# verdurin/pbdagcon

Hardware: AMD Instinct MI355X
Metric: consensus bases/sec (whole node) (higher is better)
Workload: dtype u8

## Files before the change

pbdagcon_amd/csrc/k_build.hip.h:

```cpp
#pragma once
#include <hip/hip_runtime.h>
#include "dagcon_dev.h"
#include "k_norm_run.hip.h"
#include "k_norm_fin.hip.h"

#define DG_WAVE 64
#ifndef DG_LPW
#define DG_LPW 8u
#endif

__device__ __forceinline__ bool dg_failed(const DgParams &p) {
    return __hip_atomic_load(&p.st->err_flags, __ATOMIC_RELAXED, __HIP_MEMORY_SCOPE_AGENT) != 0;
}
__device__ __forceinline__ void dg_fail(const DgParams &p, uint32_t bit) {
    atomicOr(&p.st->err_flags, bit);
}
__device__ __forceinline__ void dg_fail_target(const DgParams &p, uint32_t t, uint32_t bit) {
    atomicOr(&p.tfail[t], bit);
}
__device__ __forceinline__ bool dg_tskip(const DgParams &p, uint32_t t) {
    return !p.tactive[t] || __hip_atomic_load(&p.tfail[t], __ATOMIC_RELAXED, __HIP_MEMORY_SCOPE_AGENT) != 0;
}
__device__ __forceinline__ bool dg_askip(const DgParams &p, uint32_t a) {
    return !(p.flags & DG_F_A1_ONLY) && __hip_atomic_load(&p.tfail[p.aln_tgt[a]], __ATOMIC_RELAXED, __HIP_MEMORY_SCOPE_AGENT) != 0;
// ... 697 lines not shown
    if (p.emit_scan) {
        for (unsigned long long m = __ballot(pfx_entry); m; m = __ballot(pfx_entry)) {
            const uint32_t pp = (uint32_t)__builtin_amdgcn_readlane((int)prev_pos, __ffsll((long long)m) - 1);
            const uint32_t x = rvalid ? Cm[pp] : 0u;
            const uint32_t e = dg_wave_excl(x, lane);
            if (pfx_entry && prev_pos == pp) { prev = gbase[pp] + e + x - 1u; pfx_entry = false; }
        }
    }
    uint32_t c_base = 0x80000000u;
#define DG_STAGE(I)                                                                         \
    do {                                                                                    \
        c_base = (I) & ~7u;                                                                 \
        const uint4 *src_ = reinterpret_cast<const uint4 *>(buf + c_base);                  \
        uint4 v_[DG_ECOLS / 8];                                                             \
        _Pragma("unroll") for (int k_ = 0; k_ < (int)(DG_ECOLS / 8); k_++)                  \
            v_[k_] = (c_base + 8u * k_ < hi) ? src_[k_] : make_uint4(0, 0, 0, 0);           \
        _Pragma("unroll") for (int k_ = 0; k_ < (int)(DG_ECOLS / 8); k_++) {                \
            uint32_t *dst_ = reinterpret_cast<uint32_t *>(colw) + 4 * k_;                   \
            dst_[0] = v_[k_].x; dst_[1] = v_[k_].y; dst_[2] = v_[k_].z; dst_[3] = v_[k_].w; \
        }                                                                                   \
    } while (0)
#define DG_COLUMN(I, OUT)                                                                   \
    do {                                                                                    \
        if ((I) - c_base >= DG_ECOLS) DG_STAGE(I);                                          \
        OUT = colw[(I) - c_base];                                                           \
    } while (0)
#define DG_DEPART(NXT)                                                       \
    do {                                                                     \
        if (!(fl & DG_EF_OWN)) break;                                        \
        if (fl & DG_EF_BB) {                                                 \
            if (prev_pos >= pos0) s_D[(prev_pos - pos0) * 64 + lane] = (NXT) + 1u;   \
            else DG_ECELL(Dm, prev_pos) = (NXT) + 1u;                \
        } else {                                                             \
            const uint32_t _rk = prev - prev_pos;                            \
            DG_EPW(3u * _rk) = (NXT);                                        \
            DG_EPW(3u * _rk + 1u) = 1u;                                      \
        }                                                                    \
    } while (0)

    uint32_t pos0 = P0;
    while (pos0 < P1 && (pos0 <= blen || (!__all(bbpos == DG_EDONE) && pos0 <= blen + 2u * DG_EB))) {
        uint32_t bidv[DG_EB];
        {
            const uint4 *bp = reinterpret_cast<const uint4 *>(bid + pos0);
#pragma unroll
            for (int k = 0; k < DG_EB / 4; k++) {
                const uint4 v = bp[k];
                bidv[4 * k] = v.x; bidv[4 * k + 1] = v.y; bidv[4 * k + 2] = v.z; bidv[4 * k + 3] = v.w;
            }
        }
        uint32_t gbv[DG_EB], cmv[DG_EB];
        {
            const uint4 *gp = reinterpret_cast<const uint4 *>(gbase + pos0);
#pragma unroll
            for (int k = 0; k < DG_EB / 4; k++) {
                const uint4 v = gp[k];
                gbv[4 * k] = v.x; gbv[4 * k + 1] = v.y; gbv[4 * k + 2] = v.z; gbv[4 * k + 3] = v.w;
            }
            if constexpr (sizeof(CT) == 1) {
                const uint2 v = *reinterpret_cast<const uint2 *>(Cm + pos0);
#pragma unroll
                for (int k = 0; k < 8; k++) cmv[k] = ((k < 4 ? v.x : v.y) >> (8 * (k & 3))) & 0xFFu;
            } else {
                const uint4 *cp = reinterpret_cast<const uint4 *>(Cm + pos0);
#pragma unroll
                for (int k = 0; k < DG_EB / 4; k++) {
                    const uint4 v = cp[k];
                    cmv[4 * k] = v.x; cmv[4 * k + 1] = v.y; cmv[4 * k + 2] = v.z; cmv[4 * k + 3] = v.w;
                }
            }
        }
        if (p.emit_scan) {
#pragma unroll
            for (int j = 0; j < DG_EB; j++) {
                const uint32_t x = rvalid ? cmv[j] : 0u;
                cmv[j] = __ballot(x != 0u) ? dg_wave_excl(x, lane) : 0u;
            }
        }
        if (bbpos != DG_EDONE && i < hi && (i - c_base) + DG_ENEED > DG_ECOLS) DG_STAGE(i);
        uint32_t acell[DG_EB];
#pragma unroll
        for (int j = 0; j < DG_EB; j++) { acell[j] = 0; s_D[j * 64 + lane] = 0; }
        uint32_t exit_val = 0;
#pragma unroll
        for (int j = 0; j < DG_EB; j++) {
            const uint32_t pos = pos0 + j;
            uint32_t f_apos = 0, f_key = 0, f_first = 0;
            asm volatile("" : "+v"(fl));
            if (bbpos == pos && pos < P1) {
                uint32_t ins_id = 0;
                uint32_t kacc = 0;
                uint16_t c = 0;
                f_apos = prev_pos;
                const bool f_anc_ok = fl == (DG_EF_BB | DG_EF_OWN) && pos - prev_pos < 16u;
                for (;;) {
                    if (i < hi) DG_COLUMN(i, c);
                    const uint8_t qb = DG_Q(c), tb = DG_T(c);
                    if (i >= hi || qb == tb || qb == DG_GAP) break;
                    if (tb == DG_GAP) {
                        if (!ins_id) { ins_id = gbv[j] + cmv[j]; f_first = ins_id; }
                        kacc = (kacc << 8) | qb;
                        const uint32_t id = ins_id++;
                        const uint32_t rk = id - bbpos;
                        DgNode nd;
                        nd.out_len = 1; nd.in_len = 1; nd.base = qb; nd.flags = 0; nd.pad = 0;
                        nd.weight = 1; nd.pending = 1;
                        nd.out_off = 3u * rk; nd.in_off = 3u * rk + 2u; nd.out_cap = 1; nd.in_cap = 1;
                        nd.bbpos = (int32_t)bbpos;
                        *reinterpret_cast<DgNode *>(reinterpret_cast<char *>(ndt) + (id << 5)) = nd;
                        DG_EPW(3u * rk + 2u) = prev;
                        DG_DEPART(id);
                        prev = id; prev_pos = bbpos; fl = DG_EF_OWN;
                    }
                    i++;
                }
                if (i >= hi) {
                    exit_val = (fl & DG_EF_OWN) ? prev + 1u : 0u;
                    const uint32_t ex = bid[exitpos];
                    DG_DEPART(ex);
                    bbpos = DG_EDONE;
                } else {
                    const uint8_t qb = DG_Q(c), tb = DG_T(c);
                    if (qb == tb) {
                        const uint32_t cur = bidv[j];
                        acell[j] = ((uint32_t)tb << 25) | (prev + 1u);
                        if (f_anc_ok && kacc != 0u && kacc < (1u << 24)) f_key = kacc | ((pos - f_apos) << 24);
                        DG_DEPART(cur);
                        prev = cur; prev_pos = bbpos; fl = DG_EF_BB | DG_EF_OWN;
                    } else {
                        acell[j] = ((uint32_t)tb << 25) | DG_CELL_DEL;
                    }
                    bbpos++;
                    i++;
                }
            }
            if (p.fold) {
                const unsigned long long em = __ballot(f_key != 0u);
                if (em & (em - 1ull)) {
                    uint32_t fn;
                    const uint32_t vic = dg_emit_fold(em, f_key, f_first, pos, ndt, pool, &fn, lane);
                    if (vic | fn) {
                        const uint32_t dv = vic ? 0u : (f_first + 1u) | ((fn - 1u) << 25);
                        if (f_apos >= pos0) s_D[(f_apos - pos0) * 64 + lane] = dv;
                        if (f_apos < pos0 || f_apos == 0u) DG_ECELL(Dm, f_apos) = dv;
                        if (vic) acell[j] = (acell[j] & 0xFE000000u) | DG_CELL_DUP;
                    }
                }
            }
        }
        if (r < K && lane < DG_ERPW) {
#pragma unroll
            for (int j = 0; j < DG_EB; j++) {
                const uint32_t pos = pos0 + j;
                if (pos <= blen && pos >= P0 && pos < P1) {
                    DG_ECELL(Am, pos) = acell[j];
                    const uint32_t dv = s_D[j * 64 + lane];
                    if (pos > 0 || dv) DG_ECELL(Dm, pos) = dv;
                }
            }
            if (exit_val) DG_ECELL(Am, exitpos) = exit_val;
        }
        pos0 += DG_EB;
    }
    {
        const bool ahead = bbpos != DG_EDONE && (fl & DG_EF_OWN);
        uint32_t q = bbpos, nxt = 0;
        bool found = false, pfx_next = false;
        if (ahead) {
            while (i < hi) {
                const uint16_t c = buf[i];
                const uint8_t qb = DG_Q(c), tb = DG_T(c);
                if (qb == tb) { nxt = bid[q]; found = true; break; }
                if (qb == DG_GAP) { q++; i++; continue; }
                if (tb == DG_GAP) {
                    if (p.emit_scan) pfx_next = true; else nxt = gbase[q] + Cm[q];
                    found = true; break;
                }
                i++;
            }
        }
        if (p.emit_scan) {
            for (unsigned long long m = __ballot(pfx_next); m; m = __ballot(pfx_next)) {
                const uint32_t pp = (uint32_t)__builtin_amdgcn_readlane((int)q, __ffsll((long long)m) - 1);
                const uint32_t x = rvalid ? Cm[pp] : 0u;
                const uint32_t e = dg_wave_excl(x, lane);
                if (pfx_next && q == pp) { nxt = gbase[pp] + e; pfx_next = false; }
            }
        }
        if (ahead) {
            if (!found) {
                nxt = bid[exitpos];
                Am[(uint64_t)exitpos * K + r] = prev + 1u;
            }
            const uint32_t pos0 = 0xFFFFFFFFu;
            DG_DEPART(nxt);
        }
    }
#undef DG_EPW
#undef DG_ECELL
#undef DG_DEPART
#undef DG_COLUMN
#undef DG_STAGE
}

#include "k_lists_row.hip.h"
__device__ __forceinline__ int dg_lds_find(volatile int32_t *vals, int n, int x, int lane) {
    for (int b = 0; b < n; b += DG_WAVE) {
        int i = b + lane;
        bool hit = (i < n) && (vals[i] == x);
        unsigned long long m = __ballot(hit);
        if (m) return b + (__ffsll((long long)m) - 1);
    }
    return -1;
}

__device__ __forceinline__ uint32_t dg_pool_alloc(const DgParams &p, uint32_t t, uint32_t words, int lane) {
    uint32_t off = 0;
    if (lane == 0) {
        t = (uint32_t)__builtin_amdgcn_readfirstlane((int)t);
        off = atomicAdd(&p.pool_top[t], words);
        if ((uint64_t)off + words > p.pool_size[t]) { dg_fail(p, DG_E_POOL_TGT); p.st->bad_target = t; off = 0xFFFFFFFFu; }
    }
    return (uint32_t)__builtin_amdgcn_readlane((int)off, 0);
}

__device__ __forceinline__ unsigned long long dg_list_row(int32_t val, int32_t extra, int32_t chain, int32_t ulo, int32_t uhi,
                                                          int lane, int32_t &cnt, unsigned long long &cm) {
    cm = __ballot(val == chain);
    const bool uniq = val >= ulo && val < uhi;
    unsigned long long firsts = __ballot(uniq);
    cnt = 1 + extra;
    unsigned long long rem = __ballot(val != 0 && !uniq) & ~cm;
    while (rem) {
        const int first = __ffsll((long long)rem) - 1;
        const int32_t x = __builtin_amdgcn_readlane(val, first);
        const unsigned long long same = __ballot(val == x);
        rem &= ~same;
        if (lane == first) cnt = __popcll(same) + extra;
        firsts |= 1ull << first;
    }
    return firsts;
}

struct DgPosLists { uint32_t o_len, o_off, o_cap, i_len, i_off, i_cap, cov; };

__device__ __forceinline__ bool dg_lists_pos(const DgParams &p, uint32_t t, uint32_t *pool, uint32_t pos, uint32_t blen,
                                             uint32_t capb, uint32_t fixed0, int lane, bool do_out, bool do_in,
                                             uint32_t dep, uint32_t arr, int32_t v1, int32_t chain_o, int32_t ulo_o,
                                             int32_t chain_i, int32_t ulo_i, DgPosLists &r) {
#define DG_LPOOL(OFF) (*reinterpret_cast<uint32_t *>(reinterpret_cast<char *>(pool) + (((uint32_t)(OFF)) << 2)))
    if (do_out) {
        const int32_t val = (int32_t)DG_CELL_ID(dep), extra = (int32_t)(dep >> 25);
        int32_t cnt;
        unsigned long long cm;
        const unsigned long long firsts = dg_list_row(val, extra, chain_o, ulo_o, chain_o, lane, cnt, cm);
        const uint32_t n = 1u + (uint32_t)__popcll(firsts);
        uint32_t off = fixed0 + pos * 3u * capb, cap = capb;
        if (n > capb) {
            cap = n + 2u;
            off = dg_pool_alloc(p, t, 2u * cap, lane);
            if (off == 0xFFFFFFFFu) return false;
        }
        const uint32_t idx = 1u + (uint32_t)__popcll(firsts & ((1ull << lane) - 1ull));
        if (lane == 0) { DG_LPOOL(off) = (uint32_t)(chain_o - 1); DG_LPOOL(off + 1) = (uint32_t)__popcll(cm); }
        if ((firsts >> lane) & 1ull) { DG_LPOOL(off + 2 * idx) = (uint32_t)(val - 1); DG_LPOOL(off + 2 * idx + 1) = (uint32_t)cnt; }
        r.o_len = n; r.o_off = off; r.o_cap = cap;
    }
    if (do_in) {
        const uint32_t idf = DG_CELL_ID(arr);
        r.cov = 0;
        if (pos <= blen) {
            const unsigned long long covered = __ballot(arr != 0u);
            const uint32_t n_cov = (uint32_t)__popcll(covered);
            const uint32_t n_match = (uint32_t)__popcll(__ballot(arr != 0u && idf != DG_CELL_DEL));
            const uint32_t last_base = covered ? DG_CELL_BASE((uint32_t)__builtin_amdgcn_readlane((int)arr, 63 - __clzll((long long)covered))) : 0u;
            r.cov = n_cov | n_match << 8 | last_base << 16;
        }
        const int32_t val = (arr != 0u && idf != DG_CELL_DEL && idf != DG_CELL_DUP) ? (int32_t)idf : 0;
        int32_t cnt;
        unsigned long long cm;
        const unsigned long long firsts = dg_list_row(val, 0, chain_i, ulo_i, v1, lane, cnt, cm);
        const uint32_t n = 1u + (uint32_t)__popcll(firsts);
        uint32_t off = fixed0 + pos * 3u * capb + 2u * capb, cap = capb;
        if (n > capb) {
            cap = n + 2u;
            off = dg_pool_alloc(p, t, cap, lane);
            if (off == 0xFFFFFFFFu) return false;
        }
        const uint32_t idx = 1u + (uint32_t)__popcll(firsts & ((1ull << lane) - 1ull));
        if (lane == 0) DG_LPOOL(off) = (uint32_t)(chain_i - 1);
        if ((firsts >> lane) & 1ull) DG_LPOOL(off + idx) = (uint32_t)(val - 1);
        r.i_len = n; r.i_off = off; r.i_cap = cap;
    }
#undef DG_LPOOL
    return true;
}

__device__ __forceinline__ uint32_t dg_pool_alloc_lane(const DgParams &p, uint32_t t, uint32_t words) {
    const uint32_t off = atomicAdd(&p.pool_top[t], words);
    if ((uint64_t)off + words > p.pool_size[t]) { dg_fail(p, DG_E_POOL_TGT); p.st->bad_target = t; return 0xFFFFFFFFu; }
    return off;
}

__device__ __forceinline__ void dg_stage_rows(uint32_t *rows, const uint32_t *blk, uint32_t nrows, uint32_t K, uint32_t S,
                                              int lane) {
    if (K == 0) return;
    const uint32_t total = nrows * K, q = DG_WAVE / K, rm = DG_WAVE % K;
    uint32_t row = (uint32_t)lane / K, col = (uint32_t)lane % K;
#pragma unroll 4
    for (uint32_t i = (uint32_t)lane; i < total; i += DG_WAVE) {
        rows[row * S + col] = blk[i];
        row += q; col += rm;
        if (col >= K) { col -= K; row++; }
    }
}

#define DG_LL_WAVES 2u

__global__ __launch_bounds__(64 * DG_LL_WAVES) void k_lists_lanes(DgParams p) {
    extern __shared__ uint32_t s_rows[];
    const uint32_t t = blockIdx.x;
    if (dg_failed(p) || dg_tskip(p, t)) return;
    const uint32_t K = (uint32_t)(p.aln_begin[t + 1] - p.aln_begin[t]);
    if (K > DG_WAVE) return;
    const uint32_t blen = p.tlen[t];
    const int lane = threadIdx.x & 63;
    const uint32_t wave = (uint32_t)__builtin_amdgcn_readfirstlane((int)(threadIdx.x >> 6));
    const uint32_t pos0 = (blockIdx.y * DG_LL_WAVES + wave) * DG_WAVE;
    if (pos0 >= blen + 2) return;
    const uint32_t nrows = min((uint32_t)DG_WAVE, blen + 2 - pos0);
    const uint32_t S = K | 1u;
    uint32_t *rows = s_rows + wave * DG_WAVE * (min(p.max_k, (uint32_t)DG_WAVE) | 1u);
    uint32_t *row = rows + (uint32_t)lane * S;
    const uint64_t nb = p.node_base[t];
    const uint64_t bv = p.bbv_base[t];
    const uint32_t capb = dg_capb(K);
    const uint32_t fixed0 = 3u * p.t_nins[t];
    uint32_t *pool = p.pool + p.pool_base[t];
    const uint32_t *Db = p.matD + p.mat_base[t] + (uint64_t)pos0 * K, *Ab = p.matA + p.mat_base[t] + (uint64_t)pos0 * K;

    const uint32_t pos = pos0 + (uint32_t)lane;
    const bool act = (uint32_t)lane < nrows;
    const bool do_out = act && pos <= blen, do_in = act && pos >= 1;
    const uint32_t b0 = act ? p.bid[bv + pos] : 0u;
    const uint32_t bm = do_in ? p.bid[bv + pos - 1] : 0u;
    const uint32_t bp = do_out ? p.bid[bv + pos + 1] : 0u;
    const uint32_t g0 = act ? p.gbase[bv + pos] : 0u;
    const uint32_t g1 = do_out ? p.gbase[bv + pos + 1] : 0u;
    uint32_t out_len = 0, in_len = 0, r_cov = 0;
    uint32_t r_out = fixed0 + pos * 3u * capb, r_in = r_out + 2u * capb;
    uint32_t out_cap = capb, in_cap = capb;
    bool dead = false;

    dg_stage_rows(rows, Db, nrows, K, S, lane);
    __builtin_amdgcn_fence(__ATOMIC_SEQ_CST, "workgroup");
    DgLaneRow so = {};
    if (do_out) {
        so = dg_lane_row<false>(row, K, bp + 1u, g1 + 1u, bp + 1u);
        if (!so.overflow) {
            if (so.n > capb) {
                const uint32_t off = dg_pool_alloc_lane(p, t, 2u * (so.n + 2u));
                if (off == 0xFFFFFFFFu) dead = true;
                else { r_out = off; out_cap = so.n + 2u; }
            }
            if (!dead) { pool[r_out] = bp; pool[r_out + 1u] = so.c0; out_len = so.n; }
        }
    }
    for (uint32_t j = 1; __ballot(j < out_len) != 0ull; j++)
        if (j < out_len) {
            const uint32_t e = row[j - 1u];
            pool[r_out + 2u * j] = DG_CELL_ID(e) - 1u;
            pool[r_out + 2u * j + 1u] = dg_lane_count(so, e);
        }
    __builtin_amdgcn_fence(__ATOMIC_SEQ_CST, "workgroup");

    dg_stage_rows(rows, Ab, nrows, K, S, lane);
    __builtin_amdgcn_fence(__ATOMIC_SEQ_CST, "workgroup");
    DgLaneRow si = {};
    if (do_in) {
        si = dg_lane_row<true>(row, K, bm + 1u, g0 + 1u, b0 + 1u);
        if (pos <= blen) r_cov = si.n_cov | si.n_match << 8 | si.last_base << 16;
        if (!si.overflow && !dead) {
            if (si.n > capb) {
                const uint32_t off = dg_pool_alloc_lane(p, t, si.n + 2u);
                if (off == 0xFFFFFFFFu) dead = true;
                else { r_in = off; in_cap = si.n + 2u; }
            }
            if (!dead) { pool[r_in] = bm; in_len = si.n; }
        }
    }
    for (uint32_t j = 1; __ballot(j < in_len) != 0ull; j++)
        if (j < in_len) pool[r_in + j] = DG_CELL_ID(row[j - 1u]) - 1u;

    const unsigned long long redo_o = __ballot(do_out && so.overflow != 0u), redo_i = __ballot(do_in && si.overflow != 0u);
    for (unsigned long long rem = redo_o | redo_i; rem; rem &= rem - 1ull) {
        const int pi = __ffsll((long long)rem) - 1;
        const bool ro = (redo_o >> pi) & 1ull, ri = (redo_i >> pi) & 1ull;
        const bool rl = (uint32_t)lane < K;
        const uint32_t dep = rl && ro ? Db[(uint32_t)pi * K + (uint32_t)lane] : 0u;
        const uint32_t arr = rl && ri ? Ab[(uint32_t)pi * K + (uint32_t)lane] : 0u;
        DgPosLists r;
        const bool ok = dg_lists_pos(p, t, pool, pos0 + (uint32_t)pi, blen, capb, fixed0, lane, ro, ri, dep, arr,
                                     __builtin_amdgcn_readlane((int)b0, pi) + 1,
                                     __builtin_amdgcn_readlane((int)bp, pi) + 1, __builtin_amdgcn_readlane((int)g1, pi) + 1,
                                     __builtin_amdgcn_readlane((int)bm, pi) + 1, __builtin_amdgcn_readlane((int)g0, pi) + 1, r);
        if (lane == pi) {
            if (!ok) dead = true;
            else {
                if (ro) { out_len = r.o_len; r_out = r.o_off; out_cap = r.o_cap; }
                if (ri) { in_len = r.i_len; r_in = r.i_off; in_cap = r.i_cap; r_cov = r.cov; }
            }
        }
        if (!ok) break;
    }

    if (act && !dead) {
        const bool inner = pos >= 1 && pos <= blen;
        const uint32_t n_cov = r_cov & 0xFFu, n_match = (r_cov >> 8) & 0xFFu;
        uint32_t base;
        if (pos == 0) base = '^';
        else if (pos == blen + 1) base = '$';
        else if (n_cov) base = r_cov >> 16;
        else base = p.bb ? p.bb[p.bb_off[t] + (pos - 1)] : (uint8_t)'N';
        uint4 *rec = reinterpret_cast<uint4 *>(p.nodes + nb + b0);
        rec[0] = make_uint4(out_len | in_len << 16, base | DG_NF_BACKBONE << 8,
                            inner ? 1u + n_match : 0u,
                            in_len);
        rec[1] = make_uint4(r_out, r_in, out_cap | in_cap << 16, inner ? pos : 0u);
        p.cov[bv + pos] = inner ? (int32_t)n_cov : 0;
    }
}

__global__ __launch_bounds__(256) void k_lists(DgParams p) {
    extern __shared__ int32_t s_tmp[];
    const uint32_t t = blockIdx.x;
    if (dg_failed(p) || dg_tskip(p, t)) return;
    const int lane = threadIdx.x & 63, wave = threadIdx.x >> 6;
    const uint32_t blen = p.tlen[t];
    const uint32_t K = (uint32_t)(p.aln_begin[t + 1] - p.aln_begin[t]);
    if (K <= DG_WAVE) return;
    const uint32_t stride = p.max_k + 2;
    volatile int32_t *vals = s_tmp + (size_t)wave * 2 * stride;
    volatile int32_t *cnts = vals + stride;
    const uint64_t nb = p.node_base[t];
    const uint64_t bv = p.bbv_base[t];
    uint32_t *pool = p.pool + p.pool_base[t];
    const uint32_t *Am0 = p.matA + p.mat_base[t], *Dm0 = p.matD + p.mat_base[t];
    const uint32_t capb = dg_capb(K);
    const uint32_t fixed0 = 3u * p.t_nins[t];
    for (uint32_t pi = 0; pi < DG_LPW; pi++) {
    const uint32_t pos = (blockIdx.y * 4 + wave) * DG_LPW + pi;
    if (pos >= blen + 2) return;
    const uint32_t v = p.bid[bv + pos];
    const uint32_t *Am = Am0 + (uint64_t)pos * K;
    const uint32_t *Dm = Dm0 + (uint64_t)pos * K;
    const uint32_t fixed = fixed0 + pos * 3u * capb;
    uint32_t out_off = fixed, in_off = fixed + 2u * capb;
    uint32_t out_cap = capb, in_cap = capb;
    uint32_t out_len = 0, in_len = 0;
    uint32_t n_match = 0, n_cov = 0, last_base = 0;

    for (int dir = 0; dir < 2; dir++) {
        if (dir == 0 && pos == blen + 1) continue;
        if (dir == 1 && pos == 0) continue;
        const uint32_t *row = dir == 0 ? Dm : Am;
        int n = 1;
        int32_t lv = dir == 0 ? (int32_t)p.bid[bv + pos + 1] : (int32_t)p.bid[bv + pos - 1];
        int32_t lc = 0;
        bool in_lds = false;
        for (uint32_t r0 = 0; r0 < K; r0 += DG_WAVE) {
            const uint32_t r = r0 + lane;
            const uint32_t cell = r < K ? row[r] : 0u;
            int32_t val = (int32_t)DG_CELL_ID(cell);
            const int32_t extra = dir == 0 ? (int32_t)(cell >> 25) : 0;
            if (dir == 1) {
                const uint32_t idf = DG_CELL_ID(cell);
                const unsigned long long covered = __ballot(cell != 0u);
                if (pos <= blen) {
                    n_cov += (uint32_t)__popcll(covered);
                    n_match += (uint32_t)__popcll(__ballot(cell != 0u && idf != DG_CELL_DEL));
                    if (covered) last_base = DG_CELL_BASE((uint32_t)__builtin_amdgcn_readlane((int)cell, 63 - __clzll((long long)covered)));
                }
                val = (cell != 0u && idf != DG_CELL_DEL && idf != DG_CELL_DUP) ? (int32_t)idf : 0;
            }
            unsigned long long rem = __ballot(val != 0);
            if (!in_lds) {
                const int32_t chain = __builtin_amdgcn_readlane(lv, 0) + 1;
                const unsigned long long cm = __ballot(val == chain);
                if (lane == 0) lc += __popcll(cm);
                rem &= ~cm;
            }
            while (rem) {
                const int first = __ffsll((long long)rem) - 1;
                const int32_t x = __builtin_amdgcn_readlane(val, first);
                const unsigned long long same = __ballot(val == x);
                rem &= ~same;
                const int c = __popcll(same) + __builtin_amdgcn_readlane(extra, first);
                if (!in_lds) {
                    const unsigned long long hit = __ballot(lane < n && lv == x - 1);
                    if (hit) {
                        if (lane == __ffsll((long long)hit) - 1) lc += c;
                    } else if (n < DG_WAVE) {
                        if (lane == n) { lv = x - 1; lc = c; }
                        n++;
                    } else {
                        vals[lane] = lv; cnts[lane] = lc;
                        in_lds = true;
                    }
                }
                if (in_lds) {
                    const int idx = dg_lds_find(vals, n, x - 1, lane);
                    if (idx >= 0) {
                        if (lane == 0) cnts[idx] += c;
                    } else {
                        if (lane == 0) { vals[n] = x - 1; cnts[n] = c; }
                        n++;
                    }
                }
            }
        }
        if (n > 65000) { if (lane == 0) dg_fail_target(p, t, DG_E_INTERNAL); return; }
        uint32_t off = dir == 0 ? out_off : in_off;
        if ((uint32_t)n > capb) {
            const uint32_t cap = (uint32_t)n + 2u;
            off = dg_pool_alloc(p, t, dir == 0 ? 2u * cap : cap, lane);
            if (off == 0xFFFFFFFFu) return;
            if (dir == 0) { out_off = off; out_cap = cap; } else { in_off = off; in_cap = cap; }
        }
        if (!in_lds) {
            if (lane < n) {
                if (dir == 0) { pool[off + 2 * lane] = (uint32_t)lv; pool[off + 2 * lane + 1] = (uint32_t)lc; }
                else pool[off + lane] = (uint32_t)lv;
            }
        } else {
            for (int i = lane; i < n; i += DG_WAVE) {
                if (dir == 0) { pool[off + 2 * i] = (uint32_t)vals[i]; pool[off + 2 * i + 1] = (uint32_t)cnts[i]; }
                else pool[off + i] = (uint32_t)vals[i];
            }
        }
        if (dir == 0) out_len = (uint32_t)n; else in_len = (uint32_t)n;
    }
    if (lane == 0) {
        const bool inner = pos >= 1 && pos <= blen;
        DgNode nd;
        nd.out_len = (uint16_t)out_len;
        nd.in_len = (uint16_t)in_len;
        nd.flags = DG_NF_BACKBONE; nd.pad = 0;
        if (pos == 0) nd.base = '^';
        else if (pos == blen + 1) nd.base = '$';
        else if (n_cov) nd.base = (uint8_t)last_base;
        else nd.base = p.bb ? p.bb[p.bb_off[t] + (pos - 1)] : (uint8_t)'N';
        nd.weight = inner ? 1 + (int32_t)n_match : 0;
        nd.pending = (int32_t)in_len;
        nd.out_off = out_off; nd.in_off = in_off;
        nd.out_cap = (uint16_t)out_cap; nd.in_cap = (uint16_t)in_cap;
        nd.bbpos = inner ? (int32_t)pos : 0;
        p.cov[bv + pos] = inner ? (int32_t)n_cov : 0;
        p.nodes[nb + v] = nd;
    }
    }
}
```

pbdagcon_amd/csrc/k_merge.hip.h:

```cpp
#pragma once
#include <hip/hip_runtime.h>
#include "dagcon_dev.h"

struct DgGraph {
    DgNode *nd;
    int32_t *queue;
    uint32_t *pool;
    uint32_t pool_size;
    uint32_t *pool_top;
    int32_t *stk;
    uint32_t stk_words;
    DgStatus *st;
    uint32_t *tfail;
    uint32_t t;
    int err;
    int sh;
    int X;
    const uint32_t *sh_tab;
    uint32_t seg;
    uint32_t lg_cap;
    uint32_t *lg_cnt;
};

__device__ __forceinline__ void dgg_fail(DgGraph &g, uint32_t bit) {
// ... 308 lines not shown
#define DG_H_INLEN(h)  ((int)((h).x >> 16))
#define DG_H_BASE(h)   ((int)((h).y & 0xffu))
#define DG_H_WEIGHT(h) ((int)(h).z)
#define DG_H_PEND(h)   ((int)(h).w)
#define DG_H2_OUTOFF(h) ((h).x)
#define DG_H2_INOFF(h)  ((h).y)
#define DG_H2_OUTCAP(h) ((int)((h).z & 0xffffu))
#define DG_H2_INCAP(h)  ((int)((h).z >> 16))

#define DG_RL(v, l) __builtin_amdgcn_readlane((int)(v), (int)(l))

__device__ __forceinline__ int dg_wave_incl_scan(int v, int lane) {
    for (int o = 1; o < 64; o <<= 1) {
        const int up = __shfl_up(v, o);
        if (lane >= o) v += up;
    }
    return v;
}
struct DgWave {
    typedef unsigned long long mask;
    static constexpr int W = 64;
    static constexpr bool row_text = false;
    static __device__ __forceinline__ mask ballot(bool p) { return __ballot(p); }
    static __device__ __forceinline__ int rl(int v, int l) { return DG_RL(v, l); }
    static __device__ __forceinline__ int ffs(mask m) { return __ffsll((long long)m); }
    static __device__ __forceinline__ int popc(mask m) { return __popcll(m); }
    static __device__ __forceinline__ mask lt(int lane) { return DG_LT(lane); }
};

template <class G>
__device__ __forceinline__ int dg_sum_masked(int v, typename G::mask m) {
    int acc = 0;
    while (m) {
        const int f = G::ffs(m) - 1;
        acc += G::rl(v, f);
        m &= m - 1;
    }
    return acc;
}

template <class G>
__device__ __forceinline__ int dg_pick_group(typename G::mask cand, int base, int last, int lane,
                                             typename G::mask *mask) {
    typedef typename G::mask gmask;
    int best = 256;
    gmask bm = 0;
    const int key = ((cand >> lane) & 1) ? base : -1 - lane;
    while (cand) {
        const int f = G::ffs(cand) - 1;
        const int b = G::rl(key, f);
        const gmask same = G::ballot(key == b);
        if (b > last && b < best && G::popc(same) >= 2) { best = b; bm = same; }
        cand &= ~same;
    }
    *mask = bm;
    return best;
}

template <class G>
__device__ __forceinline__ uint32_t dg_group_alloc(DgGraph &g, uint32_t words, int lane) {
    uint32_t off = 0;
    if (lane == 0) { DgGraph gs = g; off = dgg_alloc(gs, words); }
    off = (uint32_t)G::rl((int)off, 0);
    if (off == 0xFFFFFFFFu) g.err = true;
    return off;
}

template <class G>
__device__ inline void dg_in_rewrite(DgGraph &g, int v, int vid, typename G::mask vm, int app,
                                     int pend_delta, int lane) {
    typedef typename G::mask gmask;
    const uint4 h = dg_lo16(&DG_NV(g, v)), h2 = dg_hi16(&DG_NV(g, v));
    const int len = DG_H_INLEN(h);
    uint32_t off = DG_H2_INOFF(h2);
    int cap = DG_H2_INCAP(h2);
    int e = -1;
    if (lane < len) e = (int)DG_PW(g, off + lane);
    bool rm = false;
    for (gmask m = vm; m; m &= m - 1) rm |= (e == G::rl(vid, G::ffs(m) - 1));
    const bool keep = lane < len && !rm;
    const gmask km = G::ballot(keep);
    int nlen = G::popc(km);
    const int nidx = G::popc(km & G::lt(lane));
    if (app >= 0 && nlen + 1 > cap) {
        uint32_t ncap = 2u * (uint32_t)(nlen + 1);
        if (ncap < 4) ncap = 4;
        const uint32_t noff = dg_group_alloc<G>(g, ncap, lane);
        if (noff == 0xFFFFFFFFu) return;
        off = noff; cap = (int)ncap;
    }
    if (keep) DG_PW(g, off + nidx) = (uint32_t)e;
    if (app >= 0) { if (lane == 0) DG_PW(g, off + nlen) = (uint32_t)app; nlen++; }
    if (lane == 0) {
        DgNode *n = &DG_NV(g, v);
        n->in_len = (uint16_t)nlen; n->in_off = off; n->in_cap = (uint16_t)cap;
        if (pend_delta) n->pending = DG_H_PEND(h) + pend_delta;
    }
}

template <class G>
__device__ inline bool dg_merge_out_group(DgGraph &g, int u, uint32_t u_out_off, typename G::mask M,
                                          int d, int &cnt, uint4 h, bool valid_out, int lane) {
    typedef typename G::mask gmask;
    const int an_lane = G::ffs(M) - 1;
    const gmask vm = M & ~((gmask)1 << an_lane);
    const int an = G::rl(d, an_lane);
    const bool member = (M >> lane) & 1;
    uint4 h2 = make_uint4(0, 0, 0, 0);
    if (member) h2 = dg_hi16(&DG_NV(g, d));
    int L = 0, src = -1, e = 0;
    uint32_t src_off = 0;
    {
        gmask mm = M;
        while (mm) {
            const int ml = G::ffs(mm) - 1;
            mm &= mm - 1;
            const int mlen = G::rl(DG_H_OUTLEN(h), ml);
            const uint32_t moff = (uint32_t)G::rl((int)DG_H2_OUTOFF(h2), ml);
            if (lane >= L && lane < L + mlen) { src = ml; e = lane - L; src_off = moff; }
            L += mlen;
        }
    }
    if (L > G::W) return false;
    const bool fl = lane < L;
    int n2 = -1, c2 = 0;
    if (fl) { n2 = (int)DG_PW(g, src_off + 2 * e); c2 = (int)DG_PW(g, src_off + 2 * e + 1); }
    const bool vic_entry = fl && src != an_lane;
    uint4 hn2 = make_uint4(0, 0, 0, 0);
    if (vic_entry) hn2 = dg_lo16(&DG_NV(g, n2));
    if (G::ballot(vic_entry && DG_H_INLEN(hn2) > G::W)) return false;
    if (g.sh && G::ballot(vic_entry && ((hn2.y >> 8) & DG_NF_SHARED))) return false;

    const int add_cnt = dg_sum_masked<G>(cnt, vm);
    const int add_w = dg_sum_masked<G>(DG_H_WEIGHT(h), vm);
    gmask rem = G::ballot(fl), first_m = 0;
    gmask vics = 0;
    if constexpr (G::row_text) vics = G::ballot(vic_entry);
    int newcnt = c2;
    while (rem) {
        const int f = G::ffs(rem) - 1;
        const int x = G::rl(n2, f);
        const gmask same = G::ballot(fl && n2 == x);
        rem &= ~same;
        first_m |= (gmask)1 << f;
        const int tot = dg_sum_masked<G>(c2, same);
        if (lane == f) newcnt = tot;
        if constexpr (!G::row_text) vics = G::ballot(vic_entry);
        const gmask vsame = same & vics;
        const int nv = G::popc(vsame);
        if (nv) {
            const bool is_new = (vsame >> f) & 1;
            dg_in_rewrite<G>(g, x, d, vm, is_new ? an : -1, -(nv - (is_new ? 1 : 0)), lane);
            if (g.err) return true;
        }
    }
    {
        const int nlen = G::popc(first_m);
        uint32_t off = (uint32_t)G::rl((int)DG_H2_OUTOFF(h2), an_lane);
        int cap = G::rl(DG_H2_OUTCAP(h2), an_lane);
        if (nlen > cap) {
            uint32_t ncap = 2u * (uint32_t)(nlen + 1);
            if (ncap < 4) ncap = 4;
            const uint32_t noff = dg_group_alloc<G>(g, 2u * ncap, lane);
            if (noff == 0xFFFFFFFFu) return true;
            off = noff; cap = (int)ncap;
        }
        if ((first_m >> lane) & 1) {
            const int idx = G::popc(first_m & G::lt(lane));
            DG_PW(g, off + 2 * idx) = (uint32_t)n2;
            DG_PW(g, off + 2 * idx + 1) = (uint32_t)newcnt;
        }
        const int an_w = G::rl(DG_H_WEIGHT(h), an_lane);
        if (lane == 0) {
            DgNode *a = &DG_NV(g, an);
            a->out_len = (uint16_t)nlen; a->out_off = off; a->out_cap = (uint16_t)cap;
            a->weight = an_w + add_w;
        }
    }
    {
        const bool keep = valid_out && !((vm >> lane) & 1);
        const gmask km = G::ballot(keep);
        if (keep) {
            const int idx = G::popc(km & G::lt(lane));
            DG_PW(g, u_out_off + 2 * idx) = (uint32_t)d;
            if (lane == an_lane) cnt += add_cnt;
            DG_PW(g, u_out_off + 2 * idx + 1) = (uint32_t)cnt;
        }
        if (lane == 0) DG_NV(g, u).out_len = (uint16_t)G::popc(km);
    }
    if ((vm >> lane) & 1) {
        DgNode *vn = &DG_NV(g, d);
        vn->out_len = 0; vn->in_len = 0; vn->flags |= DG_NF_DELETED;
    }
    return true;
}

template <class G>
__device__ inline bool dg_merge_in_group(DgGraph &g, int n, uint32_t n_in_off, typename G::mask M,
                                         int s, uint4 h, bool valid_in, int lane, int *an_out) {
    typedef typename G::mask gmask;
    const int an_lane = G::ffs(M) - 1;
    const gmask vm = M & ~((gmask)1 << an_lane);
    const int an = G::rl(s, an_lane);
    *an_out = an;
    const bool member = (M >> lane) & 1;
    const bool victim = (vm >> lane) & 1;
    uint4 h2 = make_uint4(0, 0, 0, 0);
    if (member) h2 = dg_hi16(&DG_NV(g, s));
    int c0 = 0;
    if (member) c0 = (int)DG_PW(g, DG_H2_OUTOFF(h2) + 1);
    int L = 0, e = 0;
    uint32_t src_off = 0;
    {
        gmask mm = vm;
        while (mm) {
            const int ml = G::ffs(mm) - 1;
            mm &= mm - 1;
            const int mlen = G::rl(DG_H_INLEN(h), ml);
            const uint32_t moff = (uint32_t)G::rl((int)DG_H2_INOFF(h2), ml);
            if (lane >= L && lane < L + mlen) { e = lane - L; src_off = moff; }
            L += mlen;
        }
    }
    if (L > G::W) return false;
    const bool fl = lane < L;
    int n1 = -1;
    if (fl) n1 = (int)DG_PW(g, src_off + e);
    uint4 hn1 = make_uint4(0, 0, 0, 0);
    if (fl) hn1 = dg_lo16(&DG_NV(g, n1));
    if (G::ballot(fl && DG_H_OUTLEN(hn1) > G::W)) return false;
    if (g.sh && G::ballot(fl && ((hn1.y >> 8) & DG_NF_SHARED))) return false;
    int a_in_len = 0;
    if constexpr (G::row_text) a_in_len = G::rl(DG_H_INLEN(h), an_lane);

    const int add_cnt = dg_sum_masked<G>(c0, vm);
    const int add_w = dg_sum_masked<G>(DG_H_WEIGHT(h), vm);
    if (lane == an_lane) {
        DG_PW(g, DG_H2_OUTOFF(h2) + 1) = (uint32_t)(c0 + add_cnt);
        DG_NV(g, an).weight = DG_H_WEIGHT(h) + add_w;
    }
    uint32_t a_in_off = (uint32_t)G::rl((int)DG_H2_INOFF(h2), an_lane);
    int a_in_cap = G::rl(DG_H2_INCAP(h2), an_lane);
    if constexpr (!G::row_text) a_in_len = G::rl(DG_H_INLEN(h), an_lane);
    bool a_dirty = false;
    gmask rem = G::ballot(fl);
    while (rem) {
        const int f = G::ffs(rem) - 1;
        const int x = G::rl(n1, f);
        rem &= ~G::ballot(fl && n1 == x);
        const uint4 hx2 = dg_hi16(&DG_NV(g, x));
        const int xlen = G::rl(DG_H_OUTLEN(hn1), f);
        const uint32_t xoff = DG_H2_OUTOFF(hx2);
        int dst = -1, c = 0;
        if (lane < xlen) { dst = (int)DG_PW(g, xoff + 2 * lane); c = (int)DG_PW(g, xoff + 2 * lane + 1); }
        bool isv = false;
        for (gmask m = vm; m; m &= m - 1) isv |= (dst == G::rl(s, G::ffs(m) - 1));
        const gmask vmask = G::ballot(lane < xlen && isv);
        const int csum = dg_sum_masked<G>(c, vmask);
        const gmask apos = G::ballot(lane < xlen && dst == an);
        const bool keep = lane < xlen && !isv;
        const gmask km = G::ballot(keep);
        int nlen = G::popc(km);
        if (keep) {
            const int idx = G::popc(km & G::lt(lane));
            DG_PW(g, xoff + 2 * idx) = (uint32_t)dst;
            DG_PW(g, xoff + 2 * idx + 1) = (uint32_t)(((apos >> lane) & 1) ? c + csum : c);
        }
        if (!apos) {
            if (lane == 0) { DG_PW(g, xoff + 2 * nlen) = (uint32_t)an; DG_PW(g, xoff + 2 * nlen + 1) = (uint32_t)csum; }
            nlen++;
            if (a_in_len + 1 > a_in_cap) {
                uint32_t ncap = 2u * (uint32_t)(a_in_len + 1);
                if (ncap < 4) ncap = 4;
                const uint32_t noff = dg_group_alloc<G>(g, ncap, lane);
                if (noff == 0xFFFFFFFFu) return true;
                int i = lane;
                if constexpr (!G::row_text) { if (lane < a_in_len) DG_PW(g, noff + lane) = DG_PW(g, a_in_off + lane); i += G::W; }
                for (; i < a_in_len; i += G::W) DG_PW(g, noff + i) = DG_PW(g, a_in_off + i);
                a_in_off = noff; a_in_cap = (int)ncap;
            }
            if (lane == 0) DG_PW(g, a_in_off + a_in_len) = (uint32_t)x;
            a_in_len++;
            a_dirty = true;
        }
        if (lane == 0) DG_NV(g, x).out_len = (uint16_t)nlen;
    }
    if (a_dirty && lane == 0) {
        DgNode *a = &DG_NV(g, an);
        a->in_len = (uint16_t)a_in_len; a->in_off = a_in_off; a->in_cap = (uint16_t)a_in_cap;
    }
    {
        const bool keep = valid_in && !victim;
        const gmask km = G::ballot(keep);
        if (keep) DG_PW(g, n_in_off + G::popc(km & G::lt(lane))) = (uint32_t)s;
        if (lane == 0) DG_NV(g, n).in_len = (uint16_t)G::popc(km);
    }
    if (victim) {
        DgNode *vn = &DG_NV(g, s);
        vn->out_len = 0; vn->in_len = 0; vn->flags |= DG_NF_DELETED;
    }
    return true;
}

__global__ __launch_bounds__(64) void k_cuts(DgParams p) {
    const uint32_t t = blockIdx.x;
    if (dg_failed(p) || dg_tskip(p, t)) return;
    const int lane = threadIdx.x;
    uint32_t *row = p.cuts + (uint64_t)t * (p.seg_max + 2u);
    const uint32_t blen = p.tlen[t];
    const DgNode *nd = p.nodes + p.node_base[t];
    const uint32_t *pool = p.pool + p.pool_base[t];
    const uint32_t *bid = p.bid + p.bbv_base[t];
    const DgNode en = nd[0];
    int kg = 0;
    for (int i = lane; i < en.out_len; i += 64) kg += (int)pool[en.out_off + 2 * i + 1];
    for (int o = 32; o; o >>= 1) kg += __shfl_xor(kg, o);
    for (int which = 0; which < 2; which++) {
        const uint32_t smax = which == 0 ? p.seg_max : p.bp_max;
        uint32_t *out = which == 0 ? row : p.cuts_bp + (uint64_t)t * (p.bp_max + 2u);
        const uint32_t smin = which == 0 ? p.seg_min : (p.seg_min + 2u) / 3u;
        uint32_t want = blen / (smin ? smin : 1u);
        if (want > smax) want = smax;
        if (want < 1) want = 1;
        uint32_t nseg = 1;
        if (lane == 0) out[1] = 0;
        for (uint32_t s = 1; s < want; s++) {
            const uint32_t p0 = 1u + (uint32_t)((uint64_t)s * blen / want);
            const uint32_t span = blen / want / 2u;
            uint32_t found = 0;
            for (uint32_t o = 0; o < span && !found; o += 64) {
                const uint32_t pos = p0 + o + (uint32_t)lane;
                uint32_t v = 0;
                bool ok = false;
                if (o + (uint32_t)lane < span && pos >= 1 && pos <= blen) {
                    v = bid[pos];
                    ok = nd[v].weight - 1 == kg;
                }
                const unsigned long long m = __ballot(ok);
                if (m) found = (uint32_t)DG_RL(v, __ffsll((long long)m) - 1);
            }
            if (found) { if (lane == 0) out[1 + nseg] = found; nseg++; }
        }
        if (lane == 0) { out[0] = nseg; if (which == 0 && !p.gcuts) atomicAdd(&p.st->n_mseg, nseg); }
    }
}

#define DG_IN_STACK 48
#define DG_QRING 256

#define DG_MM_WORKER 0
#define DG_MM_PROLOGUE 1
#define DG_MM_FINISH 2
template <bool GC = false>
__device__ __forceinline__ void dg_merge_segment(const DgParams &p, const uint32_t t, const int c_start, const int c_end,
                                                 int32_t *stk_base, const int mode = DG_MM_WORKER, const uint32_t me = 0,
                                                 const uint32_t wlo = 0, const int lvl_stop = 0) {
    const int lane = threadIdx.x & 63;
    const uint64_t nb = p.node_base[t];
    const uint32_t NT = p.n_nodes[t];
    const bool has_end = c_end != 0x7fffffff;
    const int c_hi = has_end ? c_end : (int)NT - 1;
    DgGraph g;
    const bool own_q = GC && p.gcuts && c_start == 0 && mode != DG_MM_FINISH;
    g.nd = p.nodes + nb; g.queue = own_q ? p.queue0 + nb : p.queue + nb + c_start;
    g.pool = p.pool + p.pool_base[t]; g.pool_size = p.pool_size[t]; g.pool_top = p.pool_top + t;
    g.stk = stk_base; g.stk_words = p.stk_words;
    g.st = p.st; g.tfail = p.tfail + t; g.t = t; g.err = false;
    const bool sh = GC && p.gcuts && mode == DG_MM_WORKER;
    g.sh = sh ? 1 : 0; g.X = (int)NT - 1;
    g.sh_tab = p.sh_cnt + (uint64_t)t * (2u + 2u * DG_SH_MAX); g.seg = me - wlo;
    g.lg_cap = p.sh_log; g.lg_cnt = p.seg_done + (uint64_t)me * (DG_SH_MAX + 1u);
    const int X = sh ? (int)NT - 1 : -1;
    const uint32_t N = own_q ? NT : (uint32_t)(c_hi - c_start + 1);
    __shared__ int s_stk[2 * DG_IN_STACK];
    __shared__ int s_ring[DG_QRING];
    uint32_t qh = 0, qt = 1;
    if (sh && c_start == 0) {
        qh = p.pro_state[4u * t]; qt = p.pro_state[4u * t + 1u];
        for (uint32_t i = qh + (uint32_t)lane; i < qt; i += 64) s_ring[i & (DG_QRING - 1)] = g.queue[i];
    } else if (lane == 0) { g.queue[0] = c_start; s_ring[0] = c_start; }
    DG_WAVE_FENCE();
    int lvl = 0;
    uint32_t lvl_end = 1;
    int failed = 0;
    int u_next = 0;
    bool have_next = false;
    DgNode nu_next;
    nu_next.out_len = 0; nu_next.in_len = 0;
#ifdef DG_STAMPS
    unsigned long long c_fast = 0, c_slow = 0, n_fast = 0, n_slow = 0, n_scalar = 0, t_prev = clock64(), c_a = 0, c_b = 0, c_c = 0, c_grp = 0, ng_in = 0, ng_out = 0, c_odd = 0, n_odd = 0, q_a = 0, q_b = 0, q_c = 0, q_d = 0;
#endif
    while (qh < qt && !failed) {
        if (mode == DG_MM_PROLOGUE) {
            if (qh == lvl_end) { lvl++; lvl_end = qt; }
            if (lvl > lvl_stop) break;
            have_next = false;
        }
        int u;
        const bool pre = have_next;
        if (have_next) u = u_next;
        else if (qt - qh <= DG_QRING) u = __builtin_amdgcn_readfirstlane(s_ring[qh & (DG_QRING - 1)]);
        else u = __builtin_amdgcn_readfirstlane(g.queue[qh]);
        have_next = false;
        qh++;
        bool scalar = false, merged = false;
        (void)merged;
#ifdef DG_STAMPS
        unsigned long long ts_pre = 0, ts_in = 0, acc_grp = 0, n_grp_in = 0, n_grp_out = 0;
        const unsigned long long ts0 = clock64();
#endif
        if (mode != DG_MM_PROLOGUE && (u < c_start || u > c_hi)) {
            dgw_fail(g, DG_E_INTERNAL, lane);
            break;
        }
        const bool skip_in = mode == DG_MM_WORKER && c_start != 0 && u == c_start;
        const bool in_only = u == c_end;
        if (in_only && qh != qt) { dgw_fail(g, DG_E_INTERNAL, lane); break; }
        int adj = sh ? -1 : 0;
        if (mode == DG_MM_PROLOGUE && u == (int)NT - 1 && lane == 0) p.pro_state[4u * t + 3u] |= 1u;

        {
#ifdef DG_STAMPS
            const unsigned long long tq0 = clock64();
#endif
            DgNode nu;
            if (pre) nu = nu_next; else nu = DG_NV(g, u);
            const int eff_in = skip_in ? 0 : (int)nu.in_len, eff_out = in_only ? 0 : (int)nu.out_len;
            if (eff_in <= 32 && eff_out <= 32) {
#ifdef DG_STAMPS
                const unsigned long long tq1 = clock64();
#endif
                const bool is_in = lane < 32;
                const int idx = lane & 31;
                const bool valid = is_in ? idx < eff_in : idx < eff_out;
                const uint32_t ea = is_in ? nu.in_off + (uint32_t)idx : nu.out_off + 2u * (uint32_t)idx;
                int nbr = 0, cnt = 0;
                if (valid) { nbr = (int)DG_PW(g, ea); cnt = (int)DG_PW(g, ea + 1); }
#ifdef DG_STAMPS
                asm volatile("" ::"v"(nbr), "v"(cnt));
                const unsigned long long tq2 = clock64();
#endif
                uint4 h = make_uint4(0, 0, 0, 0);
                if (valid) h = dg_lo16(&DG_NV(g, nbr));
                const bool shn = sh && valid && ((h.y >> 8) & DG_NF_SHARED);
                adj = __ballot(shn) ? 1 : 0;
                if (adj) goto generic;
                const unsigned long long cand = __ballot(((h.x >> (is_in ? 0u : 16u)) & 0xffffu) == 1u);
#ifdef DG_STAMPS
                const unsigned long long tq3 = clock64();
#endif
                const unsigned long long c_in = cand & 0xffffffffull;
                unsigned long long M = 0;
                bool in_work = false;
                if (__popcll(c_in) >= 2) in_work = dg_pick_group<DgWave>(c_in, DG_H_BASE(h), -1, lane, &M) != 256;
                if (!in_work && in_only) break;
                if (!in_work) {
                    bool live = valid && !is_in;
                    int last_out = -1;
                    bool bail = false;
                    for (;;) {
                        const unsigned long long c_out = __ballot(live && DG_H_INLEN(h) == 1);
                        int b = 256;
                        if (__popcll(c_out) >= 2) b = dg_pick_group<DgWave>(c_out, DG_H_BASE(h), last_out, lane, &M);
                        if (b == 256) break;
#ifdef DG_STAMPS
                        const unsigned long long tg0 = clock64();
#endif
                        const bool okg = dg_merge_out_group<DgWave>(g, u, nu.out_off, M, nbr, cnt, h, live, lane);
#ifdef DG_STAMPS
                        c_grp += clock64() - tg0; ng_out++;
#endif
                        if (!okg) { bail = true; break; }
                        merged = true;
                        if (g.err) break;
                        last_out = b;
                        const int an_lane = __ffsll((long long)M) - 1;
                        if (((M >> lane) & 1ull) && lane != an_lane) live = false;
                        if (live) h = dg_lo16(&DG_NV(g, nbr));
                    }
                    if (!bail) {
                        if (!g.err) {
                            const int pend = DG_H_PEND(h) - 1;
                            const unsigned long long rm = __ballot(live && pend == 0);
                            if (qh < qt) {
                                if (qt - qh <= DG_QRING) { u_next = __builtin_amdgcn_readfirstlane(s_ring[qh & (DG_QRING - 1)]); have_next = true; }
                            } else if (rm) {
                                u_next = DG_RL(nbr, __ffsll((long long)rm) - 1); have_next = true;
                            }
                            if (have_next) nu_next = DG_NV(g, u_next);
                            if (live) DG_NV(g, nbr).pending = pend;
                            if (live && pend == 0) {
                                const uint32_t pos = qt + (uint32_t)__popcll(rm & DG_LT(lane));
                                if (pos < N) { g.queue[pos] = nbr; s_ring[pos & (DG_QRING - 1)] = nbr; }
                            }
                            qt += (uint32_t)__popcll(rm);
                            if (qt > N) dgw_fail(g, DG_E_INTERNAL, lane);
                        }
                        failed = g.err;
#ifdef DG_STAMPS
                        { unsigned long long now = clock64(); if (merged) { c_slow += now - t_prev; n_slow++; } else { c_fast += now - t_prev; n_fast++; c_odd += tq0 - t_prev; q_a += tq1 - tq0; q_b += tq2 - tq1; q_c += tq3 - tq2; q_d += now - tq3; } t_prev = now; }
#endif
                        continue;
                    }
                }
            }
        }

    generic:
#ifdef DG_STAMPS
        ts_pre = clock64();
#endif
        int sp = skip_in ? 0 : 1;
        int fr_n = u, fr_last = -1;
        if (adj < 0) {
            const DgNode nq = DG_NV(g, u);
            bool f = false;
            if (!skip_in) for (int i = lane; i < nq.in_len; i += 64) f |= (DG_NV(g, DG_PW(g, nq.in_off + i)).flags & DG_NF_SHARED) != 0;
            if (!in_only) for (int i = lane; i < nq.out_len; i += 64) f |= (int)DG_PW(g, nq.out_off + 2 * i) == X;
            adj = __ballot(f) ? 1 : 0;
        }
        if (adj) scalar = true;
        while (sp > 0 && !scalar) {
            const DgNode nn = DG_NV(g, fr_n);
            if (nn.in_len > 32) { scalar = true; break; }
            const bool valid = lane < nn.in_len;
            int s = 0;
            if (valid) s = (int)DG_PW(g, nn.in_off + lane);
            uint4 h = make_uint4(0, 0, 0, 0);
            if (valid) h = dg_lo16(&DG_NV(g, s));
            const unsigned long long cand = __ballot(valid && DG_H_OUTLEN(h) == 1 && !(sh && ((h.y >> 8) & DG_NF_SHARED)));
            unsigned long long M = 0;
            int b = 256;
            if (__popcll(cand) >= 2) b = dg_pick_group<DgWave>(cand, DG_H_BASE(h), fr_last, lane, &M);
            if (b == 256) {
                sp--;
                if (sp > 0) { fr_n = s_stk[2 * (sp - 1)]; fr_last = s_stk[2 * (sp - 1) + 1]; }
                continue;
            }
            if (sp >= DG_IN_STACK) { scalar = true; break; }
            int an = -1;
#ifdef DG_STAMPS
            const unsigned long long tg0 = clock64();
#endif
            if (!dg_merge_in_group<DgWave>(g, fr_n, nn.in_off, M, s, h, valid, lane, &an)) { scalar = true; break; }
#ifdef DG_STAMPS
            acc_grp += clock64() - tg0; n_grp_in++;
#endif
            merged = true;
            if (g.err) break;
            fr_last = b;
            if (lane == 0) { s_stk[2 * (sp - 1)] = fr_n; s_stk[2 * (sp - 1) + 1] = fr_last; }
            sp++;
            fr_n = an; fr_last = -1;
        }
        if (scalar && !g.err && sp > 0) {
            DG_LANE0(g, {
                dgg_merge_in(gs, fr_n);
                for (int f = sp - 2; f >= 0 && !gs.err; f--) dgg_merge_in(gs, s_stk[2 * f]);
            });
        }

#ifdef DG_STAMPS
        ts_in = clock64();
#endif
        if (in_only) break;
        bool done = false;
        if (scalar) {
            if (!g.err) DG_LANE0(g, { dgg_merge_out(gs, u); });
        }
        int last_out = -1;
        while (!done && !g.err) {
            const DgNode nu = DG_NV(g, u);
            const int out_len = nu.out_len;
            if (out_len > 64) break;
            const bool valid = lane < out_len;
            int d = 0, cnt = 0;
            if (valid) { d = (int)DG_PW(g, nu.out_off + 2 * lane); cnt = (int)DG_PW(g, nu.out_off + 2 * lane + 1); }
            uint4 h = make_uint4(0, 0, 0, 0);
            if (valid) h = dg_lo16(&DG_NV(g, d));
            if (!scalar) {
                const unsigned long long cand = __ballot(valid && DG_H_INLEN(h) == 1 && d != X);
                unsigned long long M = 0;
                int b = 256;
                if (__popcll(cand) >= 2) b = dg_pick_group<DgWave>(cand, DG_H_BASE(h), last_out, lane, &M);
                if (b != 256) {
#ifdef DG_STAMPS
                    const unsigned long long tg0 = clock64();
                    const bool okg = dg_merge_out_group<DgWave>(g, u, nu.out_off, M, d, cnt, h, valid, lane);
                    acc_grp += clock64() - tg0; n_grp_out++;
                    if (okg) {
#else
                    if (dg_merge_out_group<DgWave>(g, u, nu.out_off, M, d, cnt, h, valid, lane)) {
#endif
                        merged = true;
                        last_out = b;
                        continue;
                    }
                    DG_LANE0(g, { dgg_merge_out(gs, u); });
                    scalar = true;
                    continue;
                }
            }
            const int pend = DG_H_PEND(h) - 1;
            const bool bk = valid && d != X;
            if (bk) DG_NV(g, d).pending = pend;
            const unsigned long long rm = __ballot(bk && pend == 0);
            if (bk && pend == 0) {
                const uint32_t pos = qt + (uint32_t)__popcll(rm & DG_LT(lane));
                if (pos < N) { g.queue[pos] = d; s_ring[pos & (DG_QRING - 1)] = d; }
            }
            qt += (uint32_t)__popcll(rm);
            if (qt > N) dgw_fail(g, DG_E_INTERNAL, lane);
            done = true;
        }
        if (!done && !g.err) {
            uint32_t nqt = qt;
            DG_LANE0(g, {
                if (!scalar) dgg_merge_out(gs, u);
                const uint32_t off = gs.nd[u].out_off;
                const int len = gs.nd[u].out_len;
                for (int i = 0; i < len && !gs.err; i++) {
                    const int v = (int)gs.pool[off + 2 * i];
                    if (v == X) continue;
                    const int pend = gs.nd[v].pending - 1;
                    gs.nd[v].pending = pend;
                    if (pend == 0) {
                        if (nqt >= N) { dgg_fail(gs, DG_E_INTERNAL); break; }
                        s_ring[nqt & (DG_QRING - 1)] = v;
                        gs.queue[nqt++] = v;
                    }
                }
            });
            qt = (uint32_t)DG_RL(nqt, 0);
        }
        failed = g.err;
#ifdef DG_STAMPS
        { unsigned long long now = clock64(); if (merged || scalar) { c_slow += now - t_prev; n_slow++; n_scalar += scalar; c_a += ts_pre - ts0; c_b += ts_in - ts_pre; c_c += now - ts_in; c_grp += acc_grp; ng_in += n_grp_in; ng_out += n_grp_out; } else { c_fast += now - t_prev; n_fast++; c_odd += now - t_prev; n_odd++; } t_prev = now; }
#endif
    }
    if (mode == DG_MM_PROLOGUE && lane == 0) {
        p.pro_state[4u * t] = qh; p.pro_state[4u * t + 1u] = qt; p.pro_state[4u * t + 2u] = qh;
    }
#ifdef DG_STAMPS
    if (t == 0 && c_start == 0 && lane == 0) { p.st->dbg[0] = n_fast; p.st->dbg[1] = n_slow; p.st->dbg[2] = c_fast; p.st->dbg[3] = c_slow; p.st->dbg[4] = n_scalar; p.st->dbg[5] = c_a; p.st->dbg[6] = c_b; p.st->dbg[7] = c_c; p.st->dbg[8] = c_grp; p.st->dbg[9] = ng_in; p.st->dbg[10] = ng_out; p.st->dbg[11] = c_odd; p.st->dbg[12] = q_a; p.st->dbg[13] = q_b; p.st->dbg[14] = q_c; p.st->dbg[15] = q_d; }
// ... 325 lines not shown
```

Measured before the change: 374.9 million.

## Batch cut-point searches across lanes and prefetch alignment rows into registers

k_cuts now runs up to 32 segment cut searches per round. A first narrow probe packs 16-wide windows of several searches into one wavefront, and later full-width probes batch all open searches with their loads issued together, replacing the serial one-search-at-a-time ballot loop. In k_lists_lanes, row staging is split into a register fetch and an LDS put. The matA block is fetched into registers while the matD rows are processed, overlapping its global-load latency, and the put uses a cheaper address walk. The costs are higher register pressure from the 64-entry per-lane cell array and from the unrolled per-search arrays, plus extra speculative loads for searches that would have ended early.

```diff
diff --git a/pbdagcon_amd/csrc/k_build.hip.h b/pbdagcon_amd/csrc/k_build.hip.h
--- a/pbdagcon_amd/csrc/k_build.hip.h
+++ b/pbdagcon_amd/csrc/k_build.hip.h
@@ -1023,18 +1023,45 @@
     return off;
 }
 
-__device__ __forceinline__ void dg_stage_rows(uint32_t *rows, const uint32_t *blk, uint32_t nrows, uint32_t K, uint32_t S,
-                                              int lane) {
+struct DgLaneCells { uint32_t c[DG_WAVE], last; };
+#define DG_ROUNDS8(b) DG_ROUND((b) + 0u) DG_ROUND((b) + 1u) DG_ROUND((b) + 2u) DG_ROUND((b) + 3u) DG_ROUND((b) + 4u) DG_ROUND((b) + 5u) DG_ROUND((b) + 6u) DG_ROUND((b) + 7u)
+
+__device__ __forceinline__ void dg_rows_fetch(DgLaneCells &r, const uint32_t *blk, uint32_t total, int lane) {
+    const uint32_t *src = blk + lane;
+    const uint32_t nfull = total / DG_WAVE;
+#define DG_ROUND(n) if ((n) >= nfull) goto cut; r.c[n] = src[(n) * DG_WAVE];
+    DG_ROUNDS8(0) DG_ROUNDS8(8) DG_ROUNDS8(16) DG_ROUNDS8(24) DG_ROUNDS8(32) DG_ROUNDS8(40) DG_ROUNDS8(48) DG_ROUNDS8(56)
+#undef DG_ROUND
+cut:
+    r.last = (uint32_t)lane < total - nfull * DG_WAVE ? src[nfull * DG_WAVE] : 0u;
+}
+
+__device__ __forceinline__ void dg_rows_put(uint32_t *rows, const DgLaneCells &r, uint32_t total, uint32_t K, uint32_t S,
+                                            int lane) {
     if (K == 0) return;
-    const uint32_t total = nrows * K, q = DG_WAVE / K, rm = DG_WAVE % K;
-    uint32_t row = (uint32_t)lane / K, col = (uint32_t)lane % K;
-#pragma unroll 4
-    for (uint32_t i = (uint32_t)lane; i < total; i += DG_WAVE) {
-        rows[row * S + col] = blk[i];
-        row += q; col += rm;
-        if (col >= K) { col -= K; row++; }
-    }
-}
+    const uint32_t nfull = total / DG_WAVE, rest = total - nfull * DG_WAVE;
+    if (S == K) {
+        uint32_t *dst = rows + lane;
+#define DG_ROUND(n) if ((n) >= nfull) goto cut_odd; dst[(n) * DG_WAVE] = r.c[n];
+        DG_ROUNDS8(0) DG_ROUNDS8(8) DG_ROUNDS8(16) DG_ROUNDS8(24) DG_ROUNDS8(32) DG_ROUNDS8(40) DG_ROUNDS8(48) DG_ROUNDS8(56)
+#undef DG_ROUND
+cut_odd:
+        if ((uint32_t)lane < rest) dst[nfull * DG_WAVE] = r.last;
+        return;
+    }
+    const uint32_t rm = DG_WAVE % K, step = DG_WAVE + DG_WAVE / K;
+    uint32_t col = (uint32_t)lane % K, a = (uint32_t)lane + (uint32_t)lane / K;
+#define DG_ROUND(n)                                  \
+    if ((n) >= nfull) goto cut;                      \
+    rows[a] = r.c[n];                                \
+    col = min(col + rm, col + rm - K);               \
+    a += step + (col < rm ? 1u : 0u);
+    DG_ROUNDS8(0) DG_ROUNDS8(8) DG_ROUNDS8(16) DG_ROUNDS8(24) DG_ROUNDS8(32) DG_ROUNDS8(40) DG_ROUNDS8(48) DG_ROUNDS8(56)
+#undef DG_ROUND
+cut:
+    if ((uint32_t)lane < rest) rows[a] = r.last;
+}
+#undef DG_ROUNDS8
 
 #define DG_LL_WAVES 2u
 
@@ -1073,7 +1100,11 @@
     uint32_t out_cap = capb, in_cap = capb;
     bool dead = false;
 
-    dg_stage_rows(rows, Db, nrows, K, S, lane);
+    const uint32_t total = nrows * K;
+    DgLaneCells cells;
+    dg_rows_fetch(cells, Db, total, lane);
+    dg_rows_put(rows, cells, total, K, S, lane);
+    dg_rows_fetch(cells, Ab, total, lane);
     __builtin_amdgcn_fence(__ATOMIC_SEQ_CST, "workgroup");
     DgLaneRow so = {};
     if (do_out) {
@@ -1095,7 +1126,7 @@
         }
     __builtin_amdgcn_fence(__ATOMIC_SEQ_CST, "workgroup");
 
-    dg_stage_rows(rows, Ab, nrows, K, S, lane);
+    dg_rows_put(rows, cells, total, K, S, lane);
     __builtin_amdgcn_fence(__ATOMIC_SEQ_CST, "workgroup");
     DgLaneRow si = {};
     if (do_in) {
diff --git a/pbdagcon_amd/csrc/k_merge.hip.h b/pbdagcon_amd/csrc/k_merge.hip.h
--- a/pbdagcon_amd/csrc/k_merge.hip.h
+++ b/pbdagcon_amd/csrc/k_merge.hip.h
@@ -634,6 +634,13 @@
     return true;
 }
 
+#ifndef DG_CUTS_U
+#define DG_CUTS_U 32u
+#endif
+#ifndef DG_CUTS_R
+#define DG_CUTS_R 16u
+#endif
+static_assert(DG_CUTS_U <= 32u && DG_CUTS_U % (64u / DG_CUTS_R) == 0u, "the searches of a round fill whole narrow probes");
 __global__ __launch_bounds__(64) void k_cuts(DgParams p) {
     const uint32_t t = blockIdx.x;
     if (dg_failed(p) || dg_tskip(p, t)) return;
@@ -656,22 +663,62 @@
         if (want < 1) want = 1;
         uint32_t nseg = 1;
         if (lane == 0) out[1] = 0;
-        for (uint32_t s = 1; s < want; s++) {
-            const uint32_t p0 = 1u + (uint32_t)((uint64_t)s * blen / want);
-            const uint32_t span = blen / want / 2u;
-            uint32_t found = 0;
-            for (uint32_t o = 0; o < span && !found; o += 64) {
-                const uint32_t pos = p0 + o + (uint32_t)lane;
-                uint32_t v = 0;
-                bool ok = false;
-                if (o + (uint32_t)lane < span && pos >= 1 && pos <= blen) {
-                    v = bid[pos];
-                    ok = nd[v].weight - 1 == kg;
+        const uint32_t span = blen / want / 2u;
+        for (uint32_t s0 = 1; s0 < want; s0 += DG_CUTS_U) {
+            const uint32_t p0l = 1u + (uint32_t)((uint64_t)(s0 + (uint32_t)lane) * blen / want);
+            const uint32_t ns = min((uint32_t)DG_CUTS_U, want - s0);
+            uint32_t open = ns >= 32u ? 0xFFFFFFFFu : (1u << ns) - 1u;
+            uint32_t foundl = 0;
+            {
+                constexpr uint32_t PR = 64u / DG_CUTS_R, NP = DG_CUTS_U / PR;
+                const uint32_t j = (uint32_t)lane & (DG_CUTS_R - 1u), rw = (uint32_t)lane / DG_CUTS_R;
+                uint32_t v[NP];
+                int32_t w[NP];
+#pragma unroll
+                for (uint32_t q = 0; q < NP; q++) {
+                    const uint32_t k = q * PR + rw;
+                    const uint32_t pos = (uint32_t)__shfl((int)p0l, (int)k) + j;
+                    v[q] = k < ns && j < span && pos >= 1 && pos <= blen ? bid[pos] : 0u;
                 }
-                const unsigned long long m = __ballot(ok);
-                if (m) found = (uint32_t)DG_RL(v, __ffsll((long long)m) - 1);
-            }
-            if (found) { if (lane == 0) out[1 + nseg] = found; nseg++; }
+#pragma unroll
+                for (uint32_t q = 0; q < NP; q++) w[q] = v[q] ? nd[v[q]].weight : 0;
+#pragma unroll
+                for (uint32_t q = 0; q < NP; q++) {
+                    const unsigned long long m = __ballot(v[q] != 0u && w[q] - 1 == kg);
+#pragma unroll
+                    for (uint32_t r = 0; r < PR; r++) {
+                        const uint32_t mr = (uint32_t)(m >> (r * DG_CUTS_R)) & ((1u << DG_CUTS_R) - 1u);
+                        if (mr) {
+                            const uint32_t f = (uint32_t)DG_RL(v[q], r * DG_CUTS_R + (uint32_t)__ffs((int)mr) - 1u);
+                            if ((uint32_t)lane == q * PR + r) foundl = f;
+                            open &= ~(1u << (q * PR + r));
+                        }
+                    }
+                }
+            }
+            for (uint32_t o = DG_CUTS_R; o < span && open; o += 64) {
+                uint32_t v[DG_CUTS_U];
+                int32_t w[DG_CUTS_U];
+#pragma unroll
+                for (uint32_t k = 0; k < DG_CUTS_U; k++) {
+                    const uint32_t pos = (uint32_t)DG_RL(p0l, k) + o + (uint32_t)lane;
+                    v[k] = ((open >> k) & 1u) && o + (uint32_t)lane < span && pos >= 1 && pos <= blen ? bid[pos] : 0u;
+                }
+#pragma unroll
+                for (uint32_t k = 0; k < DG_CUTS_U; k++) w[k] = v[k] ? nd[v[k]].weight : 0;
+#pragma unroll
+                for (uint32_t k = 0; k < DG_CUTS_U; k++) {
+                    const unsigned long long m = __ballot(v[k] != 0u && w[k] - 1 == kg);
+                    if (m) {
+                        const uint32_t f = (uint32_t)DG_RL(v[k], __ffsll((long long)m) - 1);
+                        if ((uint32_t)lane == k) foundl = f;
+                        open &= ~(1u << k);
+                    }
+                }
+            }
+            const unsigned long long fm = __ballot(foundl != 0u);
+            if (foundl) out[1u + nseg + (uint32_t)__popcll(fm & ((1ull << lane) - 1ull))] = foundl;
+            nseg += (uint32_t)__popcll(fm);
         }
         if (lane == 0) { out[0] = nseg; if (which == 0 && !p.gcuts) atomicAdd(&p.st->n_mseg, nseg); }
     }
```

After: 374.9 million. No clear change (-0.0%).
